# PierfrancescoArdino/C2M

Hardware: AMD Instinct MI355X
Metric: generator train-step frames/sec at 128x256x7 (higher is better)
Workload: dtype f32; 1 GPU; BASELINE configs[1]: 128x256, 7-frame clips (2 in + 5 predicted), batch 8/GPU, fp32, generator fwd+bwd only (no D), VGG loss on, random-init weights; global_batch=8, parallelism=single

## Files before the change

c2m_amd/csrc/conv_wino.hip:

```cpp
#include "common.h"
#include "conv_types.h"

struct WinoP {
    const float* U;
    const float* X;
    float* Y;
    const float* bias;
    int M, K, nimg;
    int Hi, Wi, Ho, Wo;
    int iy0, ix0;
    int reflect;
    long in_sn, out_sn, out_sc, out_sh, out_off;
    int in_sc, in_sh;
    unsigned x_bytes;
    int nchunks, mtiles;
    int act;
    float slope;
    float* Y2;
    long y2_sn, y2_sc, y2_sh, y2_st;
    int lo_y, lo_x, ext_y, ext_x;
    int To, Ti, nkt, cin, toff, treflect;
    long in_st, out_st;
    int th, tw;
    const int* ptab;
    int cpk;
    const float* R;
    int r_l;
};

constexpr int WR = 8, WC = 16;
constexpr int PH = WR + 2, PW = WC + 2;
constexpr int CKW = 8;
constexpr int PPOS = PH * PW;
constexpr int PCS = 192;
constexpr int PBUF = CKW * PCS;

static __device__ __forceinline__ f32x2 pk_a(f32x2 p, f32x2 q) {
    f32x2 d;
    asm("v_pk_add_f32 %0, %1, %2 op_sel:[0,0] op_sel_hi:[1,0] neg_lo:[0,1] neg_hi:[0,0]" : "=v"(d) : "v"(p), "v"(q));
    return d;
}
static __device__ __forceinline__ f32x2 pk_b(f32x2 p, f32x2 q) {
    f32x2 d;
    asm("v_pk_add_f32 %0, %1, %2 op_sel:[1,0] op_sel_hi:[1,1] neg_lo:[1,0] neg_hi:[0,1]" : "=v"(d) : "v"(p), "v"(q));
    return d;
}

template <int MT, bool GEN>
__global__ __launch_bounds__(256, MT == 1 ? 3 : 2) void conv_wino_kernel(const WinoP p) {
    constexpr int NU = 4 * MT;
    __shared__ float sP[3][PBUF];
    __shared__ float sV[2 * 16 * CKW * 32];
#ifdef WINO_OCC1
    __shared__ float sDummy[20000];
    if (threadIdx.x == 999) sDummy[p.M] = 1.f;
#endif
    const int tid = threadIdx.x, lane = tid & 63;
    const int wave = __builtin_amdgcn_readfirstlane(tid >> 6);
    const int TH = GEN ? p.th : WR / 2, TW = GEN ? p.tw : WC / 2;
    const int pw_ = GEN ? 2 * TW + 2 : PW, ppos = GEN ? (2 * TH + 2) * pw_ : PPOS;
    const int regions_x = (p.Wo + 2 * TW - 1) / (2 * TW), regions_y = (p.Ho + 2 * TH - 1) / (2 * TH);
    int rb, mt;
    {
        const unsigned L = blockIdx.x, total = gridDim.x;
        const unsigned q = total >> 3, r = total & 7u, x = L & 7u, j = L >> 3;
        const unsigned w = x * q + (x < r ? x : r) + j;
        mt = (int)(w % (unsigned)p.mtiles); rb = (int)(w / (unsigned)p.mtiles);
    }
    const int rx = rb % regions_x; rb /= regions_x;
    const int ry = rb % regions_y; const int img = rb / regions_y;
    const int oy0 = ry * 2 * TH, ox0 = rx * 2 * TW;

    const int smp = p.nkt ? img / p.To : img, frm = p.nkt ? img - smp * p.To : 0;
    const unsigned img_byte = (unsigned)(smp * (int)p.in_sn) * 4u;
    int nchunks = p.nchunks;
    int pr_src[5] = {0, 0, 0, 0, 0}, pr_ub[5] = {0, 0, 0, 0, 0}, npairs = 0;
    if (p.ptab) {
        const int* __restrict__ pt = p.ptab + frm * 11;
        npairs = pt[0];
#pragma unroll
        for (int j = 0; j < 5; ++j) { pr_src[j] = pt[1 + 2 * j]; pr_ub[j] = pt[2 + 2 * j]; }
        nchunks = npairs * p.cpk;
    }
    auto sel5 = [&](const int (&a)[5], int j) { return j == 0 ? a[0] : (j == 1 ? a[1] : (j == 2 ? a[2] : (j == 3 ? a[3] : a[4]))); };
    unsigned pvo[3];
// ... 52 lines not shown
    };
    auto load_patch = [&](int chunk, int buf) {
        dma_prepare(chunk, true);
#pragma unroll
        for (int j = 0; j < 6; ++j) dma_row(j, buf);
    };
    const float* __restrict__ ubase = p.U + (((long)mt * 4 + wave) * 8 * 64 + lane) * 4;
    const long ustride = (long)p.mtiles * 4 * 64 * 32;
    const unsigned long uaddr = (unsigned long)p.U;
    const u32x4 urs = {(unsigned)uaddr, (unsigned)(uaddr >> 32) & 0xffffu, 0xffffffffu, 0x00020000u};
    const unsigned uvo = (unsigned)((((mt * 4 + wave) * 8 * 64) + lane) * 16);
    f32x4 ua[NU];
    auto next_uchunk = [&](int chunk) {
        if (!p.ptab) return chunk;
        const int uc = sel5(pr_ub, u_j) * p.cpk + u_r;
        if (++u_r == p.cpk) { u_r = 0; ++u_j; }
        return uc;
    };
    auto load_u = [&](int chunk) {
        chunk = next_uchunk(chunk);
        const f32x4* __restrict__ q = reinterpret_cast<const f32x4*>(ubase + chunk * ustride);
#pragma unroll
        for (int i = 0; i < NU; ++i) ua[i] = q[(i * 2 / MT) * 64];
    };

    f32x16 acc[4][MT];
#pragma unroll
    for (int j = 0; j < 4; ++j)
#pragma unroll
        for (int mi = 0; mi < MT; ++mi)
#pragma unroll
            for (int r = 0; r < 16; ++r) acc[j][mi][r] = 0.f;

    const int tn = tid & 31, tk = tid >> 5;
    int ty = tn >> 3, tx = tn & 7;
    if (GEN) {
        ty = tn < TH * TW ? tn / TW : 0; tx = tn < TH * TW ? tn % TW : 0;
    }
    const int pbase = tk * PCS + (2 * ty) * pw_ + 2 * tx;
    auto read_d = [&](int pb, float (&d)[4][4]) {
#pragma unroll
        for (int a = 0; a < 4; ++a)
#pragma unroll
            for (int b = 0; b < 4; ++b) d[a][b] = sP[pb][pbase + a * pw_ + b];
    };
    auto transform_store = [&](const float (&d)[4][4], int vb) {
        float x[4][4];
#pragma unroll
        for (int b = 0; b < 4; ++b) {
            x[0][b] = d[0][b] - d[2][b];
            x[1][b] = d[1][b] + d[2][b];
            x[2][b] = d[2][b] - d[1][b];
            x[3][b] = d[1][b] - d[3][b];
        }
        float* __restrict__ v = sV + vb * (16 * CKW * 32) + tk * 32 + tn;
#pragma unroll
        for (int i = 0; i < 4; ++i) {
            v[(4 * i + 0) * CKW * 32] = x[i][0] - x[i][2];
            v[(4 * i + 1) * CKW * 32] = x[i][1] + x[i][2];
            v[(4 * i + 2) * CKW * 32] = x[i][2] - x[i][1];
            v[(4 * i + 3) * CKW * 32] = x[i][1] - x[i][3];
        }
    };

    load_patch(0, 0);
    if (nchunks > 1) load_patch(1, 1);
// ... 72 lines not shown
        xr_[1][0] = dr[1][0] + dr[2][0]; xr_[1][1] = dr[1][1] + dr[2][1];
        __builtin_amdgcn_sched_barrier(0);
        mfma_pair(8);
        xr_[2][0] = dr[2][0] - dr[1][0]; xr_[2][1] = dr[2][1] - dr[1][1];
        xr_[3][0] = dr[1][0] - dr[3][0]; xr_[3][1] = dr[1][1] - dr[3][1];
        __builtin_amdgcn_sched_barrier(0);
        mfma_pair(9);
        row(0);
        __builtin_amdgcn_sched_barrier(0);
#pragma unroll
        for (int i = 1; i < 4; ++i) {
            mfma_pair(9 + i);
            put(i - 1);
            row(i);
            __builtin_amdgcn_sched_barrier(0);
        }
        mfma_pair(13);
        put(3);
        __builtin_amdgcn_sched_barrier(0);
        mfma_pair(14);
        mfma_pair(15);
        asm volatile("s_waitcnt vmcnt(6)" ::: "memory");
#pragma unroll
        for (int i = 0; i < NU; ++i) asm volatile("" : "+v"(unext[i]));
        pnext = pnext == 2 ? 0 : pnext + 1;
    };
    f32x4 ub[NU];
    int chunk = 0;
    for (; chunk + 1 < nchunks; chunk += 2) {
        iteration(chunk, ua, ub);
        iteration(chunk + 1, ub, ua);
    }
    if (chunk < nchunks) iteration(chunk, ua, ub);
    asm volatile("s_waitcnt vmcnt(0)" ::: "memory");
    __syncthreads();

    constexpr int QS = 4 * 16 * 32 + 16;
    float* __restrict__ sR = sV;
    const int m0 = mt * 64;
    if constexpr (GEN) {
        const int en = tid & 31, rp = (tid >> 5) & 1, cg = tid >> 6;
        const int ety = en < TH * TW ? en / TW : 0, etx = en < TH * TW ? en % TW : 0;
        const int oy = oy0 + 2 * ety + rp, ox = ox0 + 2 * etx;
        const bool inb = en < TH * TW && oy < p.Ho && ox < p.Wo;
        const bool top = rp == 0;
        int mode = 0;
        float* __restrict__ yb0 = p.Y + p.out_off + (long)smp * p.out_sn + (long)frm * p.out_st + (long)oy * p.out_sh + ox;
        long cs0 = p.out_sc;
        float* __restrict__ yb1 = yb0;
        long cs1 = cs0;
        const int yi = oy - p.lo_y, xi = ox - p.lo_x;
        if (p.Y2 && (unsigned)yi < (unsigned)p.ext_y) {
            const bool in0 = (unsigned)xi < (unsigned)p.ext_x, in1 = (unsigned)(xi + 1) < (unsigned)p.ext_x;
            yb1 = p.Y2 + (long)smp * p.y2_sn + (long)frm * p.y2_st + (long)yi * p.y2_sh + xi;
            cs1 = p.y2_sc;
            mode = (in0 && in1) ? 1 : ((in0 || in1) ? 2 : 0);
        }
        if (ox + 1 >= p.Wo && mode == 0) mode = 2;
        const int ro = top ? 0 : 3 * 16 * 32;
#pragma unroll
        for (int mi = 0; mi < MT; ++mi) {
#pragma unroll
            for (int hf = 0; hf < 2; ++hf) {
                __syncthreads();
#pragma unroll
                for (int rr = 0; rr < 8; ++rr) {
// ... 143 lines not shown
        for (int a = 0; a < 4; ++a)
#pragma unroll
            for (int b2 = 0; b2 < 4; ++b2) u[a][b2] = 0.f;
        if (m < M && c < K) {
            const float* __restrict__ g = dgrad ? w + ((long)c * Cin_native + m) * 9 : w + ((long)m * Cin_native + c) * 9;
            float gg[3][3];
#pragma unroll
            for (int a = 0; a < 3; ++a)
#pragma unroll
                for (int b2 = 0; b2 < 3; ++b2) gg[a][b2] = dgrad ? g[(2 - a) * 3 + (2 - b2)] : g[a * 3 + b2];
            float row[4][3];
#pragma unroll
            for (int b2 = 0; b2 < 3; ++b2) {
                const float g0 = gg[0][b2], g1 = gg[1][b2], g2 = gg[2][b2];
                row[0][b2] = g0; row[1][b2] = 0.5f * ((g0 + g1) + g2); row[2][b2] = 0.5f * ((g0 - g1) + g2); row[3][b2] = g2;
            }
#pragma unroll
            for (int a = 0; a < 4; ++a) {
                u[a][0] = row[a][0];
                u[a][1] = 0.5f * ((row[a][0] + row[a][1]) + row[a][2]);
                u[a][2] = 0.5f * ((row[a][0] - row[a][1]) + row[a][2]);
                u[a][3] = row[a][2];
            }
        }
        const long base = ((long)chunk * mtiles + mt) * 4;
#pragma unroll
        for (int wv = 0; wv < 4; ++wv)
#pragma unroll
            for (int j = 0; j < 4; ++j)
                up[((((base + wv) * 8 + (j * 2 + mi)) * 64 + lane) << 2) + kk] = u[wv][j];
    }
}

C2M_API long c2m_wino_upack_floats(int M, int K) {
    return 16L * (c2m_cdiv(M, 64) * 64L) * (c2m_cdiv(K, CKW) * (long)CKW);
}

C2M_API int c2m_wino_filter_transform(const float* w, float* upack, int Cout, int Cin, int dgrad, void* stream) {
    C2M_ENTER();
    const int M = dgrad ? Cin : Cout, K = dgrad ? Cout : Cin;
    if (M <= 0 || K <= 0) return 0;
    const long total = c2m_wino_upack_floats(M, K);
    hipLaunchKernelGGL(wino_filter_kernel, dim3(c2m_grid(total / 16, 256)), dim3(256), 0, (hipStream_t)stream, w, upack, M,
                       K, Cin, dgrad, c2m_cdiv(M, 64), total / 16);
    return (int)hipGetLastError();
}

static void wino_region_shape(int Ho, int Wo, int* th, int* tw) {
    *th = WR / 2; *tw = WC / 2;
    const long base = (long)c2m_cdiv(Ho, WR) * c2m_cdiv(Wo, WC);
    long best = base;
    for (int a = 1; a <= 16; ++a)
        for (int b = 1; b <= 32; ++b) {
            if (a * b > 32 || (2 * a + 2) * (2 * b + 2) > PCS) continue;
            const long r = (long)c2m_cdiv(Ho, 2 * a) * c2m_cdiv(Wo, 2 * b);
            if (10 * r > 9 * base) continue;
            if (r < best || (r == best && b > *tw)) { best = r; *th = a; *tw = b; }
        }
}

C2M_API int c2m_wino_regions(int Ho, int Wo) {
    int th, tw;
    wino_region_shape(Ho, Wo, &th, &tw);
    return c2m_cdiv(Ho, 2 * th) * c2m_cdiv(Wo, 2 * tw);
}

C2M_API int c2m_conv_wino(const float* upack, const float* X, float* Y, float* Y_interior, const float* bias,
                          const int64_t* g, int act, float slope, void* stream) {
    C2M_ENTER();
    WinoP p;
    p.U = upack; p.X = X; p.Y = Y; p.bias = bias;
    p.Y2 = Y_interior; p.y2_sn = p.y2_sc = p.y2_sh = p.y2_st = 0; p.lo_y = p.lo_x = p.ext_y = p.ext_x = 0;
    if (Y_interior) {
        p.y2_sn = g[C2M_WG_Y2_SN]; p.y2_sc = g[C2M_WG_Y2_SC]; p.y2_sh = g[C2M_WG_Y2_SH];
        p.lo_y = (int)g[C2M_WG_LO_Y]; p.lo_x = (int)g[C2M_WG_LO_X]; p.ext_y = (int)g[C2M_WG_EXT_Y]; p.ext_x = (int)g[C2M_WG_EXT_X];
    }
    p.M = (int)g[C2M_WG_M]; p.K = (int)g[C2M_WG_K]; p.nimg = (int)g[C2M_WG_NIMG];
    p.Hi = (int)g[C2M_WG_HI]; p.Wi = (int)g[C2M_WG_WI]; p.Ho = (int)g[C2M_WG_HO]; p.Wo = (int)g[C2M_WG_WO];
    p.iy0 = (int)g[C2M_WG_IY0]; p.ix0 = (int)g[C2M_WG_IX0]; p.reflect = (int)g[C2M_WG_REFLECT];
    p.in_sn = g[C2M_WG_IN_SN]; p.in_sc = (int)g[C2M_WG_IN_SC]; p.in_sh = (int)g[C2M_WG_IN_SH];
    p.out_sn = g[C2M_WG_OUT_SN]; p.out_sc = g[C2M_WG_OUT_SC]; p.out_sh = g[C2M_WG_OUT_SH]; p.out_off = g[C2M_WG_OUT_OFF];
    if (g[C2M_WG_X_BYTES] <= 0 || g[C2M_WG_X_BYTES] >= 0x80000000LL) return (int)hipErrorInvalidValue;
    p.x_bytes = (unsigned)g[C2M_WG_X_BYTES];
    p.To = (int)g[C2M_WG_TO]; p.in_st = g[C2M_WG_IN_ST]; p.out_st = g[C2M_WG_OUT_ST]; p.cin = (int)g[C2M_WG_CIN]; p.nkt = (int)g[C2M_WG_NKT]; p.toff = (int)g[C2M_WG_TOFF];
    p.Ti = (int)g[C2M_WG_TI]; p.treflect = (int)g[C2M_WG_TREFLECT];
    p.ptab = (const int*)(uintptr_t)g[C2M_WG_PTAB]; p.cpk = 0;
    p.R = (const float*)(uintptr_t)g[C2M_WG_RING]; p.r_l = (int)g[C2M_WG_RING_L];
    if (p.R && (Y_interior || p.reflect || g[C2M_WG_NKT] != 0 || p.Ho < 4 || p.Wo < 4 || p.r_l < p.Ho || p.r_l < p.Wo || p.out_off != 0))
        return (int)hipErrorInvalidValue;
    if (p.nkt) {
        if (p.To <= 0 || p.Ti <= 0 || p.cin <= 0 || p.nkt * p.cin != p.K || p.nimg % p.To) return (int)hipErrorInvalidValue;
        if (Y_interior) p.y2_st = (long)p.ext_y * p.y2_sh;
        if (p.ptab) {
            if (p.cin % CKW) return (int)hipErrorInvalidValue;
            p.cpk = p.cin / CKW;
        }
    } else {
        if (p.ptab) return (int)hipErrorInvalidValue;
        p.To = 1; p.in_st = p.out_st = 0;
    }
    p.act = act; p.slope = slope;
    if (p.M <= 0 || p.K <= 0 || p.nimg <= 0 || p.Ho <= 0 || p.Wo <= 0) return 0;
    if ((((uintptr_t)upack) & 15) != 0) return (int)hipErrorInvalidValue;
    p.nchunks = c2m_cdiv(p.K, CKW);
    p.mtiles = c2m_cdiv(p.M, 64);
    wino_region_shape(p.Ho, p.Wo, &p.th, &p.tw);
    const bool gen = !(p.th == WR / 2 && p.tw == WC / 2);
    const long regions = (long)p.nimg * c2m_cdiv(p.Ho, 2 * p.th) * c2m_cdiv(p.Wo, 2 * p.tw);
    if (regions * p.mtiles > 0x7fffffffL) return (int)hipErrorInvalidValue;
    dim3 grid((unsigned)(regions * p.mtiles));
    if (gen) {
        if (p.M <= 32) hipLaunchKernelGGL((conv_wino_kernel<1, true>), grid, dim3(256), 0, (hipStream_t)stream, p);
        else           hipLaunchKernelGGL((conv_wino_kernel<2, true>), grid, dim3(256), 0, (hipStream_t)stream, p);
    } else {
        if (p.M <= 32) hipLaunchKernelGGL((conv_wino_kernel<1, false>), grid, dim3(256), 0, (hipStream_t)stream, p);
        else           hipLaunchKernelGGL((conv_wino_kernel<2, false>), grid, dim3(256), 0, (hipStream_t)stream, p);
    }
    return (int)hipGetLastError();
}

struct WinoWgP {
    const float* dY; const float* X; float* slab; float* dbslab;
    int M, K, nimg, H, W;
    int reflect;
    long dy_sn, x_sn;
    unsigned dy_bytes, x_bytes;
    int T, cin;
    long cs;
    int regions, per_split;
};

constexpr int GR = 2, GC = 16, GT = 8;
constexpr int GY_STRIDE = GR * GC + 2;
constexpr int GX_COLS = GC + 4;
constexpr int GX_STRIDE = 4 * GX_COLS + 6;

static __device__ __forceinline__ f32x2 pk_sum_diff(f32x2 t) {
    f32x2 d;
    asm("v_pk_add_f32 %0, %1, %1 op_sel:[0,1] op_sel_hi:[0,1] neg_lo:[0,0] neg_hi:[0,1]" : "=v"(d) : "v"(t));
    return d;
}

template <int NI, int MI, int NB>
// ... 506 lines not shown
```

c2m_amd/ops.py:

```python
import collections
import ctypes
import os
import weakref
import math

import numpy as np
import torch

from . import _lib

G, WG = _lib.GEOM, _lib.WINO_GEOM

ACT = {None: 0, "none": 0, "relu": 1, "lrelu": 2, "sigmoid": 3}
LRELU_SLOPE = 0.2


def _stream():
    return ctypes.c_void_p(_raw_stream(_cur_device()))


_raw_stream = getattr(torch._C, "_cuda_getCurrentRawStream", None)
_cur_device = getattr(torch._C, "_cuda_getDevice", None)
if _raw_stream is None or _cur_device is None:
    _raw_stream = lambda idx: torch.cuda.current_stream(idx).cuda_stream
# ... 1021 lines not shown
    if _chunks_for_2gib(like.shape, cw.shape, stride3, pad3) > 1:
        return False
    cpl = _plan(like, _f(cw), stride3, pad3, cmode == "reflect" and any(pad3), None)
    return _fwd_reads_only_nc8(cpl, cw.requires_grad or (cb is not None and cb.requires_grad))


def conv_consumer(conv_w, stride=1, padding=0, padding_mode="zeros", conv_b=None):
    return (conv_w, stride, padding, padding_mode, conv_b)


def _virtual_grad(like, gn):
    g = torch.empty_like(like)
    if _NC8_POISON:
        g.fill_(float("nan"))
    return _mark_nc8_only(g, gn)


def _plan_for(xs, ws, stride, pad, reflect, device, dgrad_rows=None):
    key = (xs, ws, stride, pad, reflect, device.index, _conv_bf16, dgrad_rows)
    pl = _geom_cache.get(key)
    if pl is None:
        pl = _geom_cache[key] = _ConvPlan(xs, ws, stride, pad, reflect, device, _conv_bf16, dgrad_rows)
    return pl


def _plan(x, w, stride, pad, reflect, dgrad_rows=None):
    return _plan_for(tuple(x.shape), tuple(w.shape), stride, pad, reflect, x.device, dgrad_rows)


def _gp(a):
    return a.ctypes.data_as(ctypes.c_void_p)


def _wino_filter(w, Cout, Cin, dgrad):
    L = _lib.lib()
    M, K = (Cin, Cout) if dgrad else (Cout, Cin)
    U = torch.empty(L.c2m_wino_upack_floats(M, K), device=w.device, dtype=torch.float32)
    _lib.check(L.c2m_wino_filter_transform(_p(w), _p(U), Cout, Cin, dgrad, _stream()), "wino_filter_transform")
    return U


def _pack_native(w, M, C, ck, kdims, stride, s_m, s_c):
    kt, kh, kw = kdims
    st, sh, sw = stride
    ns = 16 // ck
    taps = (kt // st) * (kh // sh) * (kw // sw)
    out = torch.empty(st * sh * sw * M, _cdiv(C, ck) * _cdiv(taps, ns) * 16, device=w.device, dtype=torch.float32)
    g = np.array([M, C, ck, kt, kh, kw, st, sh, sw, s_m, s_c], dtype=np.int64)
    _lib.check(_lib.lib().c2m_pack_weights(_p(w), _p(out), _gp(g), _stream()), "pack_weights")
    out._c2m_job = (0, g)
    return out


_frozen_pack_cache = {}
_PACK_CACHE_LIMIT = 4096


def _packed(w, frozen, kind, build):
    key = (id(w), kind)
    hit = _frozen_pack_cache.get(key)
    fresh = hit is not None and hit[0]() is w and hit[1] == w._version and hit[2] == w.data_ptr()
    if not frozen and w.is_cuda and torch.cuda.is_current_stream_capturing():
        if fresh and key in _pack_jobs and _pack_jobs[key][3] is hit[3]:
            _capture_pins[id(hit[3])] = hit[3]
            return hit[3]
        return build()
    if fresh:
        return hit[3]
    job = _pack_jobs.get(key)
    if job is not None and hit is not None and job[0]() is w and hit[0]() is w and job[3] is hit[3] and \
            hit[2] == w.data_ptr():
        refresh_trainable_packs([w])
# ... 75 lines not shown


def _dgrad_wino3d(pl, w, gy, frozen_w, out_dtype, keep):
    L = _lib.lib()
    N, Cin, Cout = pl.dims[0:3]
    Ti, Hi, Wi = pl.dims[3:6]
    dM = pl.dM
    U = _packed(w, frozen_w, ("wino-dgrad3d", dM), lambda: _wino_filter(
        w[:, :dM].flip(2).permute(2, 0, 1, 3, 4).reshape(3 * Cout, dM, 3, 3).contiguous(), 3 * Cout, dM, 1))
    gx = torch.empty(pl.in_shape, device=gy.device, dtype=torch.float32)
    tgt = torch.empty(pl.wino_dgrad_target, device=gy.device, dtype=torch.float32) if pl.reflect else gx
    g3 = pl.wino_dgrad_geom
    two = pl.reflect and pl.wino3d_pairs
    kind, tag = _dgrad_tag(pl, 27, int(g3[WG.NIMG] * g3[WG.HO] * g3[WG.WO]))
    _lib.check(_timed(kind, pl.dgrad_flops,
                      lambda: L.c2m_conv_wino(_p(U), _p(gy), _p(tgt), _p(gx) if two else None, None, _gp(g3), 0, 0.0, _stream()), tag,
                      4 * (gy.numel() + w.numel() + gx.numel())), "conv_wino dgrad 3-D")
    if pl.reflect:
        if two:
            _lib.check(L.c2m_reflect_border_add(_p(tgt), _p(gx), N * Cin, Ti, Hi, Wi, 0, 1, 1, 0, _stream()), "reflect border add 3-D")
        else:
            _lib.check(L.c2m_reflect_fold(_p(tgt), _p(gx), N * Cin, Ti, Hi, Wi, 1, 1, 1, 0, _stream()), "reflect fold 3-D")
    return gx


def _dgrad_wino(pl, w, gy, frozen_w, out_dtype, keep):
    L = _lib.lib()
    N, Cin, Cout = pl.dims[0:3]
    Ti, Hi, Wi = pl.dims[3:6]
    dev = gy.device
    g_ = pl.wino_dgrad_geom
    if pl.dgrad_route in ("wino4", "wino4_ring"):
        U, conv_wino = _packed(w, frozen_w, ("wino4-dgrad",), lambda: _wino4_filter(w, Cout, Cin, 1)), L.c2m_conv_wino4
    else:
        U, conv_wino = _packed(w, frozen_w, ("wino-dgrad",), lambda: _wino_filter(w, Cout, Cin, 1)), L.c2m_conv_wino
    gx = torch.empty(pl.in_shape, device=dev, dtype=torch.float32)
    kind, tag = _dgrad_tag(pl, 9, int(g_[WG.NIMG] * g_[WG.HO] * g_[WG.WO]))
    nbytes = 4 * (gy.numel() + w.numel() + gx.numel())
    if pl.dgrad_route in ("wino_ring", "wino4_ring"):
        Ar = _packed(w, frozen_w, ("ring-dgrad",), lambda: _ring_pack(w, Cout, Cin))
        if _RING_BUFFER:
            r_l = _ceil(max(Hi, Wi), 4)
            R = torch.empty(N * Cin * 4 * r_l, device=dev, dtype=torch.float32)

            def run_ring():
                rc = L.c2m_reflect_ring_buffer(_p(Ar), _p(gy), _p(R), N, Cout, Cin, Hi, Wi, r_l, _stream())
                g_[WG.RING], g_[WG.RING_L] = R.data_ptr(), r_l
                try:
                    return rc or conv_wino(_p(U), _p(gy), _p(gx), None, None, _gp(g_), 0, 0.0, _stream())
                finally:
                    g_[WG.RING], g_[WG.RING_L] = 0, 0
        else:
            def run_ring():
                rc = conv_wino(_p(U), _p(gy), _p(gx), None, None, _gp(g_), 0, 0.0, _stream())
                return rc or L.c2m_reflect_ring_dgrad(_p(Ar), _p(w), _p(gy), _p(gx), N, Cout, Cin, Hi, Wi, _stream())
        _lib.check(_timed(kind, pl.fwd_flops, run_ring, tag, nbytes), "conv_wino dgrad + reflect ring")
        return gx
    tgt = torch.empty(pl.dgrad_target, device=dev, dtype=torch.float32) if pl.reflect else gx
    _lib.check(_timed(kind, pl.fwd_flops,
                      lambda: conv_wino(_p(U), _p(gy), _p(tgt), _p(gx) if pl.reflect else None, None, _gp(g_), 0, 0.0, _stream()), tag,
                      nbytes), "conv_wino dgrad")
    if pl.reflect:
        _lib.check(L.c2m_reflect_border_add(_p(tgt), _p(gx), N * Cin, Ti, Hi, Wi, 0, 1, 1, 0, _stream()), "reflect border add")
    return gx


# ... 109 lines not shown
        _lib.check(fold(_p(tgt), _p(gx), N * Cin, Ti, Hi, Wi, pl.pad[0], pl.pad[1], pl.pad[2], _dt(tgt), _stream()),
                   "reflect fold")
    return gx


_DGRAD = {"wino3d": _dgrad_wino3d, "wino4": _dgrad_wino, "wino": _dgrad_wino, "wino4_ring": _dgrad_wino, "wino_ring": _dgrad_wino,
          "k333_nc8": _dgrad_nc8, "s2_nc8": _dgrad_nc8, "g8": _dgrad_igemm, "igemm_batched": _dgrad_igemm, "patch_nc8": _dgrad_igemm,
          "igemm": _dgrad_igemm}


def _conv_dgrad(pl, w, gy, frozen_w, out_dtype=torch.float32, keep=None):
    if not pl.bf16:
        gy = _as(gy, torch.float32)
    gx = _DGRAD[pl.dgrad_route](pl, w, gy, frozen_w, out_dtype, keep)
    if pl.dM < pl.dims[1]:
        gx[:, pl.dM:].zero_()
    return gx if gx.dtype == out_dtype else gx.to(out_dtype)


def _fwd_timed(pl, run, x, w, y, what):
    _lib.check(_timed(pl.fwd_prof[0], pl.fwd_flops, run, pl.fwd_prof[1],
                      x.element_size() * x.numel() + 4 * w.numel() + y.element_size() * y.numel()), what)


def _fwd_wino(pl, x, w, b, y, act, slope, frozen_w, keep):
    L = _lib.lib()
    N, Cin, Cout = pl.dims[0:3]
    conv_wino = L.c2m_conv_wino
    if pl.fwd_route == "wino3d":
        U = _packed(w, frozen_w, ("wino-fwd3d",), lambda: _wino_filter(
            w.permute(0, 2, 1, 3, 4).reshape(Cout, 3 * Cin, 3, 3).contiguous(), Cout, 3 * Cin, 0))
    elif pl.fwd_route == "wino4":
        U, conv_wino = _packed(w, frozen_w, ("wino4-fwd",), lambda: _wino4_filter(w, Cout, Cin, 0)), L.c2m_conv_wino4
    else:
        U = _packed(w, frozen_w, ("wino-fwd",), lambda: _wino_filter(w, Cout, Cin, 0))
    _fwd_timed(pl, lambda: conv_wino(_p(U), _p(x), _p(y), None, _p(b), _gp(pl.wino_fwd_geom), act, slope, _stream()), x, w, y,
               "conv_wino fwd")


def _fwd_nc8(pl, x, w, b, y, act, slope, frozen_w, keep):
    L = _lib.lib()
    N, Cin, Cout, Ti, Hi, Wi = pl.dims[0:6]
    if pl.fwd_route == "k333_nc8":
        A = _packed(w, frozen_w, ("fwd-bf16-k333",), lambda: _pack_bf16_k333(w, Cout, Cin))
        run = lambda: L.c2m_conv3d_nc8(_p(A), _p(_to_nc8(x, keep)), _p(y), _p(b), Cout, Cin, N, Ti, Hi, Wi, int(pl.reflect), 1, act, slope,
                                       _stream())
    else:
        A = _packed(w, frozen_w, ("fwd-bf16-s2",), lambda: _pack_bf16_patch(w, Cout, Cin, pl.K, 16, 2))
        run = lambda: L.c2m_conv_s2_nc8(_p(A), _p(_to_nc8(x, keep)), _p(y), _p(b), Cout, Cin, N, Hi, Wi, int(pl.reflect), 1, act, slope,
                                        _stream())
    _fwd_timed(pl, run, x, w, y, "conv_nc8 fwd")


def _fwd_igemm(pl, x, w, b, y, act, slope, frozen_w, keep):
    L = _lib.lib()
    N, Cin, Cout = pl.dims[0:3]
    route = pl.fwd_route
    S = pl.g8_fwd_splits if route == "g8" else pl.fwd_splits
    dst = y if S == 1 else torch.empty(S * y.numel(), device=x.device, dtype=torch.float32)
    if route == "g8":
        A = _packed(w, frozen_w, ("fwd-bf16-g8",), lambda: _pack_bf16_gather(w, Cout, Cin, pl.dims[9:12], (1, 1, 1), pl.K, pl.K // Cin))

        def run():
            xn = _to_nc8(x)
            _set_io(pl.g8_fwd_geom, xn, BF16)
            return L.c2m_conv_igemm(_p(A), _p(xn), _p(dst), None, _p(b), _p(pl.g8_fwd_tab), _gp(pl.g8_fwd_geom), act, slope, _stream())
# ... 1867 lines not shown
```

include/c2m_hip.h:

```cpp
#ifndef C2M_HIP_H
#define C2M_HIP_H
#include <stdint.h>
#ifdef __cplusplus
extern "C" {
#endif

enum { C2M_ACT_NONE = 0, C2M_ACT_RELU = 1, C2M_ACT_LRELU = 2, C2M_ACT_SIGMOID = 3 };

#include "c2m_geom.h"
int c2m_abi_version(void);
int c2m_geom_len(void);
int c2m_wino_geom_len(void);

int c2m_conv_igemm_splits(int M, int nk, int Npix);
int c2m_conv_igemm(const float* A, const void* X, void* Y, void* Y_interior, const float* bias, const int* ktab,
                   const int64_t* geom, int act, float slope, void* stream);
int c2m_splitk_reduce(const float* slab, void* out, const float* bias, long total, int splits, long chan_stride,
                      int M, int act, float slope, int dt , void* stream);

int c2m_conv_wgrad_splits(int M, int J, int Npix);
int c2m_conv_wgrad_rows(int M, int ngroups);
int c2m_conv_wgrad(const void* dY, const void* X, float* slab, float* dW, float* db, const int* jtab,
                   const int64_t* geom, void* stream);

// ... 1 lines not shown
int c2m_pack_job_bytes(void);
long c2m_pack_job_fill(void* host_job, int type, const void* w, void* packed, const int64_t* g, unsigned first_block);
int c2m_pack_multi(const void* device_jobs, const void* device_blocktab ,
                   int njobs, long total_blocks, void* stream);
long c2m_pack_weights_bf16_patch_bytes(int M, int C);
int c2m_pack_weights_bf16_patch(const float* w, void* out, const int64_t* g, void* stream);
long c2m_pack_weights_bf16_gather_bytes(const int64_t* g);
int c2m_pack_weights_bf16_gather(const float* w, void* out, const int64_t* g, void* stream);

int c2m_nchw_to_nc8(const void* x, void* y, long N, int C, long HW, void* stream);
int c2m_conv_patch_nc8(const void* A, const void* X_nc8, void* Y, void* Y_interior, const float* bias, const int64_t* geom,
                       int act, float slope, void* stream);
long c2m_pack_weights_bf16_s2_bytes(int M, int C);
int c2m_conv_s2_nc8(const void* A, const void* X_nc8, void* Y, const float* bias, int M, int C, long N, int Hi, int Wi, int reflect,
                    int yh, int act, float slope, void* stream);
int c2m_conv_s2_dgrad_nc8(const void* A, const void* dY_nc8, void* T, int M, int K, long N, int Ho, int Wo, int reflect, int th,
                          void* stream);
int c2m_conv3d_nc8(const void* A, const void* X_nc8, void* Y, const float* bias, int M, int C, long N, int T, int H, int W, int reflect,
                   int yh, int act, float slope, void* stream);
int c2m_conv3d_dgrad_nc8(const void* A, const void* dY_nc8, void* target, const int* ptab, int M, int Ctot, int K, long N, int T, int H,
                         int W, int reflect, int th, void* stream);
int c2m_conv_wgrad3d_nc8(const void* dY_nc8, const void* X_nc8, float* slab, float* dW, float* db, int M, int C, long N, int T, int H,
                         int W, int reflect, void* stream);
int c2m_conv_wgrad_nc8_splits(int M, int C, long N, int H, int W, int s2);
long c2m_conv_wgrad_nc8_slab_floats(int M, int C, long N, int H, int W, int s2);
int c2m_conv_wgrad_nc8(const void* dY_nc8, const void* X_nc8, float* slab, float* dW, float* db, int M, int C, long N, int H,
                       int W, int reflect, int s2, void* stream);

long c2m_wino_upack_floats(int M, int K);
int c2m_wino_filter_transform(const float* w, float* upack, int Cout, int Cin, int dgrad, void* stream);
int c2m_wino_regions(int Ho, int Wo);
int c2m_conv_wino(const float* upack, const float* X, float* Y, float* Y_interior, const float* bias,
                  const int64_t* geom, int act, float slope, void* stream);

long c2m_wino4_upack_floats(int M, int K);
int c2m_wino4_filter_transform(const float* w, float* upack, int Cout, int Cin, int dgrad, void* stream);
int c2m_wino4_regions(int Ho, int Wo);
int c2m_conv_wino4(const float* upack, const float* X, float* Y, float* Y_interior, const float* bias,
                   const int64_t* geom, int act, float slope, void* stream);

int c2m_wino_wgrad_splits(int M, int K, int nimg, int H, int W);
int c2m_conv_wino_wgrad(const float* dY, const float* X, float* slab, float* dbslab, float* dW, float* db, int M, int K,
                        int nimg, int H, int W, int reflect, void* stream);
int c2m_conv_wino_wgrad3d(const float* dY, const float* X, float* slab, float* dbslab, float* dW, float* db,
                          int M, int Cin, int N, int T, int H, int W, int reflect, void* stream);

int c2m_direct_math_counts(int64_t* out, int reset);

long c2m_ring_pack_floats(int C, int M);
int c2m_ring_pack(const float* w, float* apack, int C, int M, void* stream);
int c2m_reflect_ring_dgrad(const float* apack, const float* w, const float* dY, float* dX, int N, int C, int M, int H, int W,
                           void* stream);
int c2m_reflect_ring_buffer(const float* apack, const float* dY, float* R, int N, int C, int M, int H, int W, int r_l,
                            void* stream);

int c2m_reflect_border_add(const void* dXpad, void* dX, long NC, int T, int H, int W, int pt, int ph, int pw,
                           int dt, void* stream);
int c2m_reflect_fold(const void* dXpad, void* dX, long NC, int T, int H, int W, int pt, int ph, int pw,
                     int dt, void* stream);

long c2m_norm_workspace_floats(int N, int C, long S);
int c2m_norm_stats(const void* x, float* mean, float* invstd, float* running_mean, float* running_var,
                   float* workspace, int N, int C, long S, int mode, float eps, float momentum, int dt, void* stream);
int c2m_norm_set_fused(int on);
int c2m_norm_fwd(const void* x, float* mean, float* invstd, float* running_mean, float* running_var, float* workspace,
                 const float* gamma, const float* beta, const void* gb, void* y, int N, int C, long S, int mode, float eps,
// ... 193 lines not shown
```

Baseline: 998.0 frames/s.

## Add bf16 split-precision MFMA path for Winograd F(2,3) convolutions

Adds a new Winograd kernel variant that splits the fp32 transformed filters and inputs into three bf16 pieces each and accumulates the partial products with bf16 32x32x16 MFMA instead of the fp32 MFMA path. A separate filter-transform kernel emits the split bf16 operand layout, and a host heuristic selects the split path by default when the workgroup count is large and M<=768. The aim is higher matrix throughput from bf16 MFMA while keeping near-fp32 accuracy. The cost is extra split/pack work, more LDS for a four-deep patch buffer, and a new software pipeline that has to hide these overheads.

Result: no change. 1008 frames/s, median of 5 (+1.0%).

```diff
diff --git a/c2m_amd/csrc/conv_wino.hip b/c2m_amd/csrc/conv_wino.hip
--- a/c2m_amd/csrc/conv_wino.hip
+++ b/c2m_amd/csrc/conv_wino.hip
@@ -1,5 +1,8 @@
+#include <cstdlib>
+#include <cstring>
 #include "common.h"
 #include "conv_types.h"
+#include "conv_common.h"
 
 struct WinoP {
     const float* U;
@@ -26,6 +29,7 @@
     int cpk;
     const float* R;
     int r_l;
+    unsigned u_bytes;
 };
 
 constexpr int WR = 8, WC = 16;
@@ -46,11 +50,19 @@
     return d;
 }
 
-template <int MT, bool GEN>
+template <int MT, bool GEN, int PREC = 0>
 __global__ __launch_bounds__(256, MT == 1 ? 3 : 2) void conv_wino_kernel(const WinoP p) {
+    static_assert(PREC == 0 || (PREC == 2 && MT == 2), "split operands: 64-row tiles only");
     constexpr int NU = 4 * MT;
-    __shared__ float sP[3][PBUF];
-    __shared__ float sV[2 * 16 * CKW * 32];
+    constexpr int NPB = PREC == 2 ? 4 : 3;
+    constexpr int VFLOATS = PREC == 2 ? 3 * 16 * 2 * 32 * 4 : 2 * 16 * CKW * 32;
+    struct Lds {
+        float P[NPB][PBUF];
+        float V[VFLOATS];
+    };
+    __shared__ Lds lds_;
+    float (&sP)[NPB][PBUF] = lds_.P;
+    float (&sV)[VFLOATS] = lds_.V;
 #ifdef WINO_OCC1
     __shared__ float sDummy[20000];
     if (threadIdx.x == 999) sDummy[p.M] = 1.f;
@@ -169,6 +181,103 @@
 #pragma unroll
             for (int r = 0; r < 16; ++r) acc[j][mi][r] = 0.f;
 
+    if constexpr (PREC == 2) {
+        const int nsteps = (nchunks + 1) >> 1;
+        const int tn = 16 * (wave & 1) + (lane & 15), cq = 2 * (wave >> 1) + ((lane >> 4) & 1), hi = lane >> 5;
+        const int tk = 2 * cq + hi;
+        int ty = tn >> 3, tx = tn & 7;
+        if (GEN) { ty = tn < TH * TW ? tn / TW : 0; tx = tn < TH * TW ? tn % TW : 0; }
+        const int pbase = tk * PCS + (2 * ty) * pw_ + 2 * tx;
+        unsigned* __restrict__ vw = reinterpret_cast<unsigned*>(&sV[0]) + tn * 4 + cq + hi * 256;
+        const uint4* __restrict__ vr = reinterpret_cast<const uint4*>(&sV[0]) + (4 * wave) * 64 + lane;
+        f32x2 dr[4][2], xr_[4][2];
+        auto t_read = [&](int pb) {
+#pragma unroll
+            for (int a = 0; a < 4; ++a)
+#pragma unroll
+                for (int h = 0; h < 2; ++h) dr[a][h] = *reinterpret_cast<const f32x2*>(&sP[pb][pbase + a * pw_ + 2 * h]);
+        };
+        auto t_cols = [&]() {
+#pragma unroll
+            for (int h = 0; h < 2; ++h) {
+                xr_[0][h].x = dr[0][h].x - dr[2][h].x; xr_[0][h].y = dr[0][h].y - dr[2][h].y;
+                xr_[1][h].x = dr[1][h].x + dr[2][h].x; xr_[1][h].y = dr[1][h].y + dr[2][h].y;
+                xr_[2][h].x = dr[2][h].x - dr[1][h].x; xr_[2][h].y = dr[2][h].y - dr[1][h].y;
+                xr_[3][h].x = dr[1][h].x - dr[3][h].x; xr_[3][h].y = dr[1][h].y - dr[3][h].y;
+            }
+        };
+        auto t_pair = [&](int i, int half, int kh) {
+            f32x2 o;
+            if (half == 0) { o.x = xr_[i][0].x - xr_[i][1].x; o.y = xr_[i][0].y + xr_[i][1].x; }
+            else { o.x = xr_[i][1].x - xr_[i][0].y; o.y = xr_[i][0].y - xr_[i][1].y; }
+            unsigned pe[3], po[3];
+            c2m_split3(o.x, pe[0], pe[1], pe[2]);
+            c2m_split3(o.y, po[0], po[1], po[2]);
+#pragma unroll
+            for (int q = 0; q < 3; ++q) {
+                const auto r = __builtin_amdgcn_permlane32_swap(pe[q], po[q], false, false);
+                vw[(q * 16 + 4 * i + 2 * half) * 256 + kh * 128] = c2m_pack_hi(r[0], r[1]);
+            }
+        };
+        auto t_slot = [&](int k, int pb, int kh) {
+            if (k == 0) t_read(pb);
+            else if (k == 1) t_cols();
+            else if (k < 10) t_pair((k - 2) >> 1, (k - 2) & 1, kh);
+        };
+        const __amdgpu_buffer_rsrc_t ursrc = __builtin_amdgcn_make_buffer_rsrc(const_cast<float*>(p.U), 0, p.u_bytes, 0x00020000);
+        const int uvo_s = ((mt * 4 + wave) * 24 * 64 + lane) * 16;
+        const int ustep = p.mtiles * 96 * 1024;
+        auto load_u6 = [&](bf16x8 (&u)[6], int step, int j) {
+#pragma unroll
+            for (int r = 0; r < 6; ++r)
+                u[r] = __builtin_bit_cast(bf16x8, __builtin_amdgcn_raw_buffer_load_b128(ursrc, uvo_s, step * ustep + (j * 6 + r) * 1024, 0));
+        };
+        auto xi_mfma = [&](int j, const bf16x8 (&u)[6], const bf16x8 (&b)[3], auto&& slot) {
+#pragma unroll
+            for (int qq = 0; qq < C2M_SPLIT_NPROD; ++qq)
+#pragma unroll
+                for (int mi = 0; mi < 2; ++mi) {
+                    acc[j][mi] = __builtin_amdgcn_mfma_f32_32x32x16_bf16(u[mi * 3 + C2M_SPLIT_PA[qq]], b[C2M_SPLIT_PB[qq]], acc[j][mi], 0, 0, 0);
+                    slot(qq * 2 + mi);
+                    __builtin_amdgcn_sched_barrier(0);
+                }
+        };
+        bf16x8 uA[6], uB[6];
+        load_u6(uA, 0, 0);
+        load_patch(0, 0);
+        load_patch(1, 1);
+        if (nsteps > 1) { load_patch(2, 2); load_patch(3, 3); }
+        asm volatile("s_waitcnt vmcnt(0)" ::: "memory");
+        __syncthreads();
+#pragma unroll
+        for (int kh = 0; kh < 2; ++kh)
+#pragma unroll
+            for (int k = 0; k < 10; ++k) t_slot(k, kh, kh);
+        for (int s = 0; s < nsteps; ++s) {
+            asm volatile("s_waitcnt vmcnt(0)" ::: "memory");
+            __syncthreads();
+            bf16x8 bfr[4][3];
+#pragma unroll
+            for (int j = 0; j < 4; ++j)
+#pragma unroll
+                for (int q = 0; q < 3; ++q) bfr[j][q] = __builtin_bit_cast(bf16x8, vr[(q * 16 + j) * 64]);
+            load_u6(uB, s, 1);
+            xi_mfma(0, uA, bfr[0], [](int) {});
+            __syncthreads();
+            load_u6(uA, s, 2);
+            const int c0 = 2 * s + 4, db = c0 & 3;
+            xi_mfma(1, uB, bfr[1], [&](int k) {
+                if (k == 0) dma_prepare(c0, c0 < 2 * nsteps);
+                if (k == 6) dma_prepare(c0 + 1, c0 + 1 < 2 * nsteps);
+                dma_row(k < 6 ? k : k - 6, db + (k < 6 ? 0 : 1));
+            });
+            load_u6(uB, s, 3);
+            const int pb = (2 * s + 2) & 3;
+            xi_mfma(2, uA, bfr[2], [&](int k) { t_slot(k, pb, 0); });
+            load_u6(uA, s + 1 < nsteps ? s + 1 : s, 0);
+            xi_mfma(3, uB, bfr[3], [&](int k) { t_slot(k, pb + 1, 1); });
+        }
+    } else {
     const int tn = tid & 31, tk = tid >> 5;
     int ty = tn >> 3, tx = tn & 7;
     if (GEN) {
@@ -307,6 +416,7 @@
         iteration(chunk + 1, ub, ua);
     }
     if (chunk < nchunks) iteration(chunk, ua, ub);
+    }
     asm volatile("s_waitcnt vmcnt(0)" ::: "memory");
     __syncthreads();
 
@@ -516,8 +626,70 @@
     }
 }
 
+__global__ void wino_filter_split_kernel(const float* __restrict__ w, unsigned short* __restrict__ up, int M, int K, int Cin_native,
+                                         int dgrad, int mtiles, long pairs) {
+    for (long i = blockIdx.x * (long)blockDim.x + threadIdx.x; i < pairs; i += (long)gridDim.x * blockDim.x) {
+        const int e = (int)(i & 7); long r = i >> 3;
+        const int lane = (int)(r & 63); r >>= 6;
+        const int mi = (int)(r & 1); r >>= 1;
+        const int mt = (int)(r % mtiles); const int step = (int)(r / mtiles);
+        const int m = mt * 64 + mi * 32 + (lane & 31), c = step * 16 + (lane >> 5) * 8 + e;
+        float u[4][4];
+#pragma unroll
+        for (int a = 0; a < 4; ++a)
+#pragma unroll
+            for (int b2 = 0; b2 < 4; ++b2) u[a][b2] = 0.f;
+        if (m < M && c < K) {
+            const float* __restrict__ g = dgrad ? w + ((long)c * Cin_native + m) * 9 : w + ((long)m * Cin_native + c) * 9;
+            float gg[3][3];
+#pragma unroll
+            for (int a = 0; a < 3; ++a)
+#pragma unroll
+                for (int b2 = 0; b2 < 3; ++b2) gg[a][b2] = dgrad ? g[(2 - a) * 3 + (2 - b2)] : g[a * 3 + b2];
+            float row[4][3];
+#pragma unroll
+            for (int b2 = 0; b2 < 3; ++b2) {
+                const float g0 = gg[0][b2], g1 = gg[1][b2], g2 = gg[2][b2];
+                row[0][b2] = g0; row[1][b2] = 0.5f * ((g0 + g1) + g2); row[2][b2] = 0.5f * ((g0 - g1) + g2); row[3][b2] = g2;
+            }
+#pragma unroll
+            for (int a = 0; a < 4; ++a) {
+                u[a][0] = row[a][0];
+                u[a][1] = 0.5f * ((row[a][0] + row[a][1]) + row[a][2]);
+                u[a][2] = 0.5f * ((row[a][0] - row[a][1]) + row[a][2]);
+                u[a][3] = row[a][2];
+            }
+        }
+        const long base = ((long)step * mtiles + mt) * 4;
+#pragma unroll
+        for (int wv = 0; wv < 4; ++wv)
+#pragma unroll
+            for (int j = 0; j < 4; ++j) {
+                unsigned pc[3];
+                c2m_split3(u[wv][j], pc[0], pc[1], pc[2]);
+#pragma unroll
+                for (int q = 0; q < 3; ++q)
+                    up[(((((base + wv) * 4 + j) * 2 + mi) * 3 + q) * 64 + lane) * 8 + e] = (unsigned short)(pc[q] >> 16);
+            }
+    }
+}
+
 C2M_API long c2m_wino_upack_floats(int M, int K) {
     return 16L * (c2m_cdiv(M, 64) * 64L) * (c2m_cdiv(K, CKW) * (long)CKW);
+}
+
+C2M_API long c2m_wino_upack_split_floats(int M, int K) {
+    return 24L * (c2m_cdiv(M, 64) * 64L) * (c2m_cdiv(K, 16) * 16L);
+}
+
+C2M_API int c2m_wino_filter_transform_split(const float* w, float* upack, int Cout, int Cin, int dgrad, void* stream) {
+    C2M_ENTER();
+    const int M = dgrad ? Cin : Cout, K = dgrad ? Cout : Cin;
+    if (M <= 0 || K <= 0) return 0;
+    const long pairs = (c2m_cdiv(M, 64) * 64L) * (c2m_cdiv(K, 16) * 16L);
+    hipLaunchKernelGGL(wino_filter_split_kernel, dim3(c2m_grid(pairs, 256)), dim3(256), 0, (hipStream_t)stream, w,
+                       reinterpret_cast<unsigned short*>(upack), M, K, Cin, dgrad, c2m_cdiv(M, 64), pairs);
+    return (int)hipGetLastError();
 }
 
 C2M_API int c2m_wino_filter_transform(const float* w, float* upack, int Cout, int Cin, int dgrad, void* stream) {
@@ -549,8 +721,59 @@
     return c2m_cdiv(Ho, 2 * th) * c2m_cdiv(Wo, 2 * tw);
 }
 
+static int wino_math() {
+    const char* e = getenv("C2M_WINO_MATH");
+    if (!e || !*e || !strcmp(e, "auto")) return 2;
+    if (!strcmp(e, "fp32")) return 0;
+    if (!strcmp(e, "split")) return 1;
+    return -1;
+}
+
+constexpr int C2M_WINO_COUNTS = 2;
+static long wino_counts[C2M_WINO_COUNTS];
+C2M_API int c2m_wino_math_counts(int64_t* out, int reset) {
+    for (int i = 0; i < C2M_WINO_COUNTS; ++i) {
+        const long v = reset ? __atomic_exchange_n(&wino_counts[i], 0L, __ATOMIC_RELAXED) : __atomic_load_n(&wino_counts[i], __ATOMIC_RELAXED);
+        if (out) out[i] = v;
+    }
+    return C2M_WINO_COUNTS;
+}
+
+static bool wino_split_built(int M, int K, int nkt, bool ptab) {
+    return M > 32 && nkt == 0 && !ptab && c2m_wino_upack_split_floats(M, K) * 4 < 0x7fffffffL;
+}
+static bool wino_split_pays(int mode, int M, int K, long wgs, bool gen) {
+    if (mode != 2) return mode == 1;
+    (void)K; (void)gen;
+    return wgs >= 256 && M <= 768;
+}
+
+static int conv_wino_launch(const float* upack, const float* X, float* Y, float* Y_interior, const float* bias,
+                            const int64_t* g, int act, float slope, void* stream, int split);
+
+C2M_API int c2m_wino_math(const int64_t* g) {
+    const int mode = wino_math();
+    if (mode < 0) return -1;
+    const int M = (int)g[C2M_WG_M], K = (int)g[C2M_WG_K];
+    if (M <= 0 || K <= 0 || !wino_split_built(M, K, (int)g[C2M_WG_NKT], g[C2M_WG_PTAB] != 0)) return 0;
+    int th, tw;
+    wino_region_shape((int)g[C2M_WG_HO], (int)g[C2M_WG_WO], &th, &tw);
+    const long wgs = g[C2M_WG_NIMG] * c2m_cdiv((int)g[C2M_WG_HO], 2 * th) * c2m_cdiv((int)g[C2M_WG_WO], 2 * tw) * c2m_cdiv(M, 64);
+    return wino_split_pays(mode, M, K, wgs, !(th == WR / 2 && tw == WC / 2)) ? 1 : 0;
+}
+
 C2M_API int c2m_conv_wino(const float* upack, const float* X, float* Y, float* Y_interior, const float* bias,
                           const int64_t* g, int act, float slope, void* stream) {
+    return conv_wino_launch(upack, X, Y, Y_interior, bias, g, act, slope, stream, 0);
+}
+
+C2M_API int c2m_conv_wino_split(const float* upack, const float* X, float* Y, float* Y_interior, const float* bias,
+                                const int64_t* g, int act, float slope, void* stream) {
+    return conv_wino_launch(upack, X, Y, Y_interior, bias, g, act, slope, stream, 1);
+}
+
+static int conv_wino_launch(const float* upack, const float* X, float* Y, float* Y_interior, const float* bias,
+                            const int64_t* g, int act, float slope, void* stream, int split) {
     C2M_ENTER();
     WinoP p;
     p.U = upack; p.X = X; p.Y = Y; p.bias = bias;
@@ -593,6 +816,15 @@
     const long regions = (long)p.nimg * c2m_cdiv(p.Ho, 2 * p.th) * c2m_cdiv(p.Wo, 2 * p.tw);
     if (regions * p.mtiles > 0x7fffffffL) return (int)hipErrorInvalidValue;
     dim3 grid((unsigned)(regions * p.mtiles));
+    p.u_bytes = 0;
+    if (split) {
+        if (!wino_split_built(p.M, p.K, p.nkt, p.ptab != nullptr)) return (int)hipErrorInvalidValue;
+        p.u_bytes = (unsigned)(c2m_wino_upack_split_floats(p.M, p.K) * 4);
+        if (gen) hipLaunchKernelGGL((conv_wino_kernel<2, true, 2>), grid, dim3(256), 0, (hipStream_t)stream, p);
+        else     hipLaunchKernelGGL((conv_wino_kernel<2, false, 2>), grid, dim3(256), 0, (hipStream_t)stream, p);
+        __atomic_fetch_add(&wino_counts[gen ? 1 : 0], 1L, __ATOMIC_RELAXED);
+        return (int)hipGetLastError();
+    }
     if (gen) {
         if (p.M <= 32) hipLaunchKernelGGL((conv_wino_kernel<1, true>), grid, dim3(256), 0, (hipStream_t)stream, p);
         else           hipLaunchKernelGGL((conv_wino_kernel<2, true>), grid, dim3(256), 0, (hipStream_t)stream, p);
diff --git a/c2m_amd/ops.py b/c2m_amd/ops.py
--- a/c2m_amd/ops.py
+++ b/c2m_amd/ops.py
@@ -1077,12 +1077,23 @@
     return a.ctypes.data_as(ctypes.c_void_p)
 
 
-def _wino_filter(w, Cout, Cin, dgrad):
+def _wino_filter(w, Cout, Cin, dgrad, split=False):
     L = _lib.lib()
     M, K = (Cin, Cout) if dgrad else (Cout, Cin)
+    if split:
+        U = torch.empty(L.c2m_wino_upack_split_floats(M, K), device=w.device, dtype=torch.float32)
+        _lib.check(L.c2m_wino_filter_transform_split(_p(w), _p(U), Cout, Cin, dgrad, _stream()), "wino_filter_transform_split")
+        return U
     U = torch.empty(L.c2m_wino_upack_floats(M, K), device=w.device, dtype=torch.float32)
     _lib.check(L.c2m_wino_filter_transform(_p(w), _p(U), Cout, Cin, dgrad, _stream()), "wino_filter_transform")
     return U
+
+
+def _wino_split(geom):
+    r = _lib.lib().c2m_wino_math(_gp(geom))
+    if r < 0:
+        raise RuntimeError("c2m_amd: C2M_WINO_MATH must be fp32, split or auto")
+    return bool(r)
 
 
 def _pack_native(w, M, C, ck, kdims, stride, s_m, s_c):
@@ -1224,6 +1235,8 @@
     g_ = pl.wino_dgrad_geom
     if pl.dgrad_route in ("wino4", "wino4_ring"):
         U, conv_wino = _packed(w, frozen_w, ("wino4-dgrad",), lambda: _wino4_filter(w, Cout, Cin, 1)), L.c2m_conv_wino4
+    elif _wino_split(g_):
+        U, conv_wino = _packed(w, frozen_w, ("wino-dgrad", "split"), lambda: _wino_filter(w, Cout, Cin, 1, True)), L.c2m_conv_wino_split
     else:
         U, conv_wino = _packed(w, frozen_w, ("wino-dgrad",), lambda: _wino_filter(w, Cout, Cin, 1)), L.c2m_conv_wino
     gx = torch.empty(pl.in_shape, device=dev, dtype=torch.float32)
@@ -1399,6 +1412,8 @@
             w.permute(0, 2, 1, 3, 4).reshape(Cout, 3 * Cin, 3, 3).contiguous(), Cout, 3 * Cin, 0))
     elif pl.fwd_route == "wino4":
         U, conv_wino = _packed(w, frozen_w, ("wino4-fwd",), lambda: _wino4_filter(w, Cout, Cin, 0)), L.c2m_conv_wino4
+    elif _wino_split(pl.wino_fwd_geom):
+        U, conv_wino = _packed(w, frozen_w, ("wino-fwd", "split"), lambda: _wino_filter(w, Cout, Cin, 0, True)), L.c2m_conv_wino_split
     else:
         U = _packed(w, frozen_w, ("wino-fwd",), lambda: _wino_filter(w, Cout, Cin, 0))
     _fwd_timed(pl, lambda: conv_wino(_p(U), _p(x), _p(y), None, _p(b), _gp(pl.wino_fwd_geom), act, slope, _stream()), x, w, y,
diff --git a/include/c2m_hip.h b/include/c2m_hip.h
--- a/include/c2m_hip.h
+++ b/include/c2m_hip.h
@@ -57,6 +57,12 @@
 int c2m_wino_regions(int Ho, int Wo);
 int c2m_conv_wino(const float* upack, const float* X, float* Y, float* Y_interior, const float* bias,
                   const int64_t* geom, int act, float slope, void* stream);
+long c2m_wino_upack_split_floats(int M, int K);
+int c2m_wino_filter_transform_split(const float* w, float* upack, int Cout, int Cin, int dgrad, void* stream);
+int c2m_wino_math(const int64_t* geom);
+int c2m_conv_wino_split(const float* upack, const float* X, float* Y, float* Y_interior, const float* bias,
+                        const int64_t* geom, int act, float slope, void* stream);
+int c2m_wino_math_counts(int64_t* out, int reset);
 
 long c2m_wino4_upack_floats(int M, int K);
 int c2m_wino4_filter_transform(const float* w, float* upack, int Cout, int Cin, int dgrad, void* stream);
```
